# latk/hbetune.rs

Measured on NVIDIA B200. Metric: gp_fit_lml_evals_per_s, higher is better.
Workload: dtype f64

## Files before the change

### hbetune_rs_b200/csrc/gemm_i8.cuh

```cuda
#pragma once
#include <cuda.h>
#include <cuda_runtime.h>
#include <stdint.h>

#include "kernels.cuh"
#include "tcgen05.cuh"

namespace hbegp {
namespace oz {

using namespace tc;

constexpr int S = 14;
__host__ __device__ constexpr int modulus(int m) {
    return m == 0 ? 256 : m == 1 ? 255 : m == 2 ? 253 : m == 3 ? 251 : m == 4 ? 247 : m == 5 ? 241 : m == 6 ? 239
         : m == 7 ? 233 : m == 8 ? 229 : m == 9 ? 227 : m == 10 ? 223 : m == 11 ? 217 : m == 12 ? 211 : 199;
}
constexpr uint64_t P_LO = 0x3bdc01086e91ad00ull, P_HI = 0x0000478ff11c7ad1ull;
constexpr uint64_t HALF_LO = 0x9dee00843748d680ull, HALF_HI = 0x000023c7f88e3d68ull;
constexpr double INV_P58 = 1.9858025962649873e-16;
__host__ __device__ constexpr uint32_t crt_limb(int m, int l) {
    constexpr uint32_t t[S][4] = {
        {0x37fb0e01u, 0x3da6cc26u, 0xcdd91dc0u, 0x00000a57u},
        {0x2d9b6200u, 0x515b4421u, 0x61efbe69u, 0x00003c0eu},
        {0x6436c700u, 0xa8c49274u, 0x2ee81407u, 0x000033c3u},
        {0x0aaff900u, 0xaff19c1cu, 0xd136bce2u, 0x00000446u},
        {0xf7471500u, 0xd3598a93u, 0xb743daa4u, 0x000032b3u},
        {0xb4ac3100u, 0x80994803u, 0x38e00b2au, 0x00003a7fu},
        {0xb50dfd00u, 0xf9cd4608u, 0xfc396104u, 0x00001c71u},
        {0x0fc58900u, 0xf5ef92cau, 0x53de92a8u, 0x00002dc3u},
        {0x2b43a200u, 0x4f7c9d74u, 0xf258b82cu, 0x0000419fu},
        {0x93d41700u, 0x4d8fc60du, 0xcd5da098u, 0x0000303bu},
        {0x1a5f8a00u, 0x9a05c78eu, 0x5ab66f28u, 0x0000421bu},
        {0x5e122800u, 0x90ded2a3u, 0x9f5e87f5u, 0x00002cd9u},
        {0xd7195400u, 0xa67b8783u, 0xca9cace9u, 0x00003a55u},
        {0x8f385a00u, 0x80e799d2u, 0x8574cdfdu, 0x00003310u},
    };
    return t[m][l];
}

constexpr int TB = 128;
constexpr int TILE_BYTES = TB * TB;
constexpr int STAGES = 3;
constexpr int THREADS = 192;
constexpr int TMEM_COLS = 128;
constexpr size_t SMEM_BYTES = (size_t)STAGES * 2 * TILE_BYTES + 1024  + 256 ;
constexpr int E_CLAMP = 400;
constexpr int E_BAD = -32768;
constexpr int MAX_BITS = 50;

inline int scale_bits(int np) {
    const unsigned __int128 half = ((unsigned __int128)HALF_HI << 64) | HALF_LO;
    int b = MAX_BITS;
    while (b > 0 && ((unsigned __int128)np << (2 * b)) >= half) --b;
    return b;
}

__host__ __device__ inline long ntri_of(int tiles) { return (long)tiles * (tiles + 1) / 2; }
inline long ntri(int np) { return ntri_of((np + TB - 1) / TB); }
inline size_t slot_bytes(int np) {
    const size_t ex = ((size_t)(np + TB - 1) / TB * TB * sizeof(int) + TILE_BYTES - 1) / TILE_BYTES * TILE_BYTES;
    return 2 * (size_t)S * ntri(np) * TILE_BYTES + ex;
}

template <int M>
__device__ __forceinline__ uint32_t residue_byte(uint32_t lo24, uint32_t h0, uint32_t h1) {
    constexpr uint32_t p = (uint32_t)modulus(M);
    constexpr uint32_t c24 = (uint32_t)((1ull << 24) % p), c36 = (uint32_t)((1ull << 36) % p);
    constexpr uint32_t off = (uint32_t)(p - (uint32_t)((1ull << 51) % p));
    const uint32_t t = lo24 + h0 * c24 + h1 * c36 + off;
    uint32_t r = t % p;
    if (r > (p - 1) / 2) r -= p;
    return r & 0xffu;
}

template <int M>
__device__ __forceinline__ void store_residues(unsigned char* dst, const uint32_t (&lo)[16], const uint32_t (&h0)[16],
                                               const uint32_t (&h1)[16]) {
    uint32_t w[4];
#pragma unroll
    for (int q = 0; q < 4; q++)
        w[q] = residue_byte<M>(lo[4 * q], h0[4 * q], h1[4 * q]) | residue_byte<M>(lo[4 * q + 1], h0[4 * q + 1], h1[4 * q + 1]) << 8 |
               residue_byte<M>(lo[4 * q + 2], h0[4 * q + 2], h1[4 * q + 2]) << 16 |
               residue_byte<M>(lo[4 * q + 3], h0[4 * q + 3], h1[4 * q + 3]) << 24;
    *reinterpret_cast<uint4*>(dst) = make_uint4(w[0], w[1], w[2], w[3]);
}

template <int M>
__device__ __forceinline__ void store_all(unsigned char* dst, size_t plane_bytes, const uint32_t (&lo)[16], const uint32_t (&h0)[16],
                                          const uint32_t (&h1)[16]) {
    store_residues<M>(dst + (size_t)M * plane_bytes, lo, h0, h1);
    if constexpr (M + 1 < S) store_all<M + 1>(dst, plane_bytes, lo, h0, h1);
}

__global__ void __launch_bounds__(512) k_oz_colexp(const double* __restrict__ W, long mstride, int np, int bits,
                                                   unsigned char* __restrict__ ws, size_t slot) {
    __shared__ double smax[512];
    const int c = blockIdx.x, b = blockIdx.z, tid = threadIdx.x, col = tid & (TB - 1), ph = tid >> 7;
    const int nt = (np + TB - 1) / TB;
    const double* Wb = W + (long)b * mstride;
    int* ex = reinterpret_cast<int*>(ws + (size_t)b * slot + 2 * (size_t)S * ntri_of(nt) * TILE_BYTES);
    const int j = c * TB + col;
    double m = 0.0;
    if (j < np) {
        for (int k = c * TB + ph; k < min(np, (c + 1) * TB); k += 4)
            if (k >= j) { const double a = fabs(Wb[(long)k * np + j]); m = (a > m || a != a) ? a : m; }
#pragma unroll 8
        for (int k = (c + 1) * TB + ph; k < np; k += 4) { const double a = fabs(Wb[(long)k * np + j]); m = (a > m || a != a) ? a : m; }
    }
    smax[tid] = m;
    __syncthreads();
    if (tid < TB) {
        for (int q = 1; q < 4; q++) { const double a = smax[tid + q * TB]; m = (a > m || a != a) ? a : m; }
        int e = 0;
        if (!(m <= 0x1p+440)) {
            e = E_BAD;
        } else if (m > 0.0) {
            int E;
            frexp(m, &E);
            e = min(max(bits - E, -E_CLAMP), E_CLAMP);
        }
        ex[j] = e;
    }
}

__global__ void __launch_bounds__(256, 2) k_oz_split(const double* __restrict__ W, long mstride, int np,
                                                     unsigned char* __restrict__ ws, size_t slot) {
    int kb, c;
    lower_tile(blockIdx.x, kb, c);
    const int b = blockIdx.z, tid = threadIdx.x, col = tid & (TB - 1), j = c * TB + col;
    const long nr = ntri_of((np + TB - 1) / TB);
    const double* Wb = W + (long)b * mstride;
    unsigned char* wsb = ws + (size_t)b * slot;
    const int e = reinterpret_cast<const int*>(wsb + 2 * (size_t)S * nr * TILE_BYTES)[j];
    const double sc = e == E_BAD ? 0.0 : __longlong_as_double((long long)(1023 + e) << 52);
    const size_t plane_bytes = (size_t)nr * TILE_BYTES;
    unsigned char* tile = wsb + (size_t)blockIdx.x * TILE_BYTES;
    constexpr double MAGIC = 0x1.8p+52;
    for (int it = tid; it < TB * (TB / 16); it += 256) {
        const int ch = it >> 7, k0 = kb * TB + ch * 16;
        uint32_t lo[16], h0[16], h1[16];
#pragma unroll
        for (int q = 0; q < 16; q++) {
            const int k = k0 + q;
            const double w = (j < np && k < np && k >= j) ? Wb[(long)k * np + j] : 0.0;
            const uint64_t u = (uint64_t)__double_as_longlong(fma(w, sc, MAGIC)) & ((1ull << 52) - 1);
            lo[q] = (uint32_t)u & 0xffffffu;
            h0[q] = (uint32_t)(u >> 24) & 0xfffu;
            h1[q] = (uint32_t)(u >> 36);
        }
        store_all<0>(tile + (size_t)col * TB + ch * 16, plane_bytes, lo, h0, h1);
    }
}

struct SyrkParams {
    CUtensorMap map;
    unsigned char* ws;
    size_t slot;
    int nt;
    int slot_tiles;
};

constexpr uint32_t IDESC = (2u << 4) | (1u << 7) | (1u << 10) | ((uint32_t)(TB >> 3) << 17) | ((uint32_t)(TB >> 4) << 24);

__device__ __forceinline__ void mma_i8(uint32_t tmem_d, uint64_t adesc, uint64_t bdesc, uint32_t accumulate) {
    asm volatile(
        "{\n\t"
        ".reg .pred p;\n\t"
        "setp.ne.b32 p, %4, 0;\n\t"
        "tcgen05.mma.cta_group::1.kind::i8 [%0], %1, %2, %3, p;\n\t"
        "}\n" ::"r"(tmem_d),
        "l"(adesc), "l"(bdesc), "r"(IDESC), "r"(accumulate)
        : "memory");
}

__global__ void __launch_bounds__(THREADS, 2) k_oz_syrk_i8(const __grid_constant__ SyrkParams p) {
    extern __shared__ unsigned char smem_raw[];
    unsigned char* smem = reinterpret_cast<unsigned char*>((reinterpret_cast<uintptr_t>(smem_raw) + 1023) & ~(uintptr_t)1023);
    uint64_t* bars = reinterpret_cast<uint64_t*>(smem + (size_t)STAGES * 2 * TILE_BYTES);
    uint64_t* full = bars;
    uint64_t* empty = bars + STAGES;
    uint64_t* accf = bars + 2 * STAGES;
    uint32_t* tmem_slot = reinterpret_cast<uint32_t*>(accf + 1);

    const int tid = threadIdx.x, warp = tid >> 5, lane = tid & 31;
    int mt, nt;
    lower_tile(blockIdx.x, mt, nt);
    const int mod = blockIdx.y, bz = blockIdx.z;
    const long nr = (long)p.nt * (p.nt + 1) / 2;
    const int nk = p.nt - mt;
    const bool diag = mt == nt;

    if (warp == 0 && lane == 0) {
        for (int s = 0; s < STAGES; s++) {
            mbar_init(&full[s], 1);
            mbar_init(&empty[s], 1);
        }
        mbar_init(accf, 1);
        asm volatile("fence.mbarrier_init.release.cluster;" ::: "memory");
        asm volatile("prefetch.tensormap [%0];" ::"l"(reinterpret_cast<uint64_t>(&p.map)) : "memory");
    }
    if (warp == 1) {
        asm volatile("tcgen05.alloc.cta_group::1.sync.aligned.shared::cta.b32 [%0], %1;" ::"r"(smem_u32(tmem_slot)), "r"(TMEM_COLS)
                     : "memory");
        asm volatile("tcgen05.relinquish_alloc_permit.cta_group::1.sync.aligned;" ::: "memory");
    }
    asm volatile("tcgen05.fence::before_thread_sync;" ::: "memory");
    __syncthreads();
    asm volatile("tcgen05.fence::after_thread_sync;" ::: "memory");
    const uint32_t tmem_base = *tmem_slot;

    if (warp == 0) {
        if (lane == 0) {
            const int z0 = bz * p.slot_tiles + mod * (int)nr;
            for (int kt = 0; kt < nk; kt++) {
                const int s = kt % STAGES, kb = mt + kt;
                mbar_wait(&empty[s], ((kt / STAGES) & 1) ^ 1);
                unsigned char* st = smem + (size_t)s * 2 * TILE_BYTES;
                const int z = z0 + kb * (kb + 1) / 2;
                mbar_expect_tx(&full[s], diag ? TILE_BYTES : 2 * TILE_BYTES);
                tma_load_3d(&p.map, &full[s], st, 0, 0, z + mt);
                if (!diag) tma_load_3d(&p.map, &full[s], st + TILE_BYTES, 0, 0, z + nt);
            }
        }
    } else if (warp == 1) {
        if (lane == 0) {
            for (int kt = 0; kt < nk; kt++) {
                const int s = kt % STAGES;
                mbar_wait(&full[s], (kt / STAGES) & 1);
                asm volatile("tcgen05.fence::after_thread_sync;" ::: "memory");
                const uint32_t a = smem_u32(smem + (size_t)s * 2 * TILE_BYTES), bb = diag ? a : a + TILE_BYTES;
#pragma unroll
                for (int ks = 0; ks < TB / 32; ks++)
                    mma_i8(tmem_base, make_desc(a + 32 * ks, 16, 1024, 2), make_desc(bb + 32 * ks, 16, 1024, 2), (kt | ks) ? 1u : 0u);
                mma_commit(&empty[s]);
            }
            mma_commit(accf);
        }
    } else {
        const int lane_base = 32 * (warp & 3), row = lane_base + lane;
        const uint32_t lane_addr = tmem_base + ((uint32_t)lane_base << 16);
        const int pm = modulus(mod);
        const float inv = 1.0f / (float)pm;
        mbar_wait(accf, 0);
        asm volatile("tcgen05.fence::after_thread_sync;" ::: "memory");
        unsigned char* dst = p.ws + (size_t)bz * p.slot + ((size_t)(S + mod) * nr + blockIdx.x) * TILE_BYTES + (size_t)row * TB;
#pragma unroll
        for (int c0 = 0; c0 < TB; c0 += 32) {
            uint32_t v[32];
            tmem_ld32(lane_addr + c0, v);
            asm volatile("tcgen05.wait::ld.sync.aligned;" ::: "memory");
            uint32_t w[8];
#pragma unroll
            for (int q = 0; q < 8; q++) {
                uint32_t packed = 0;
#pragma unroll
                for (int e = 0; e < 4; e++) {
                    const int x = (int)v[4 * q + e];
                    int r = x - (int)floorf((float)x * inv) * pm;
                    r += r < 0 ? pm : 0;
                    r -= r >= pm ? pm : 0;
                    packed |= (uint32_t)r << (8 * e);
                }
                w[q] = packed;
            }
            reinterpret_cast<uint4*>(dst + c0)[0] = make_uint4(w[0], w[1], w[2], w[3]);
            reinterpret_cast<uint4*>(dst + c0)[1] = make_uint4(w[4], w[5], w[6], w[7]);
        }
        asm volatile("tcgen05.fence::before_thread_sync;" ::: "memory");
    }
    __syncthreads();
    if (warp == 1) {
        asm volatile("tcgen05.dealloc.cta_group::1.sync.aligned.b32 %0, %1;" ::"r"(tmem_base), "r"(TMEM_COLS) : "memory");
    }
}

__device__ __forceinline__ double crt_value(const uint32_t (&r)[S], int e) {
    uint64_t acc0 = 0, acc1 = 0, acc2 = 0, acc3 = 0;
#pragma unroll
    for (int m = 0; m < S; m++) {
        acc0 += (uint64_t)r[m] * crt_limb(m, 0);
        acc1 += (uint64_t)r[m] * crt_limb(m, 1);
        acc2 += (uint64_t)r[m] * crt_limb(m, 2);
        acc3 += (uint64_t)r[m] * crt_limb(m, 3);
    }
    typedef unsigned __int128 u128;
    typedef __int128 i128;
    const u128 sum = (u128)acc0 + ((u128)acc1 << 32) + ((u128)acc2 << 64) + ((u128)acc3 << 96);
    const u128 P = ((u128)P_HI << 64) | P_LO, half = ((u128)HALF_HI << 64) | HALF_LO;
    const uint32_t q = (uint32_t)((double)(uint64_t)(sum >> 58) * INV_P58);
    i128 v = (i128)(sum - (u128)q * P);
    if (v < 0) v += (i128)P;
    if (v >= (i128)P) v -= (i128)P;
    if (v > (i128)half) v -= (i128)P;
    const bool neg = v < 0;
    const u128 a = neg ? (u128)(-v) : (u128)v;
    const uint64_t hi = (uint64_t)(a >> 64), lo = (uint64_t)a;
    double d;
    int sh = 0;
    if (hi == 0) {
        d = __ull2double_rn(lo);
    } else {
        sh = 64 - __clzll((long long)hi);
        const uint64_t mant = (uint64_t)(a >> sh) | ((lo & ((1ull << sh) - 1)) != 0 ? 1ull : 0ull);
        d = __ull2double_rn(mant);
    }
    d *= __longlong_as_double((long long)(1023 + sh - e) << 52);
    return neg ? -d : d;
}

__global__ void __launch_bounds__(256) k_oz_merge(double* __restrict__ C, long mstride, int np, const unsigned char* __restrict__ ws,
                                                  size_t slot) {
    int mt, nt;
    lower_tile(blockIdx.x, mt, nt);
    const int b = blockIdx.z, tnum = (np + TB - 1) / TB;
    const long nr = (long)tnum * (tnum + 1) / 2;
    const unsigned char* wsb = ws + (size_t)b * slot;
    const unsigned char* res = wsb + ((size_t)S * nr + blockIdx.x) * TILE_BYTES;
    const int* ex = reinterpret_cast<const int*>(wsb + 2 * (size_t)S * nr * TILE_BYTES);
    double* Cb = C + (long)b * mstride;
    for (int it = threadIdx.x; it < TB * TB / 4; it += 256) {
        const int row = it >> 5, c4 = (it & 31) * 4;
        const int gi = mt * TB + row, gj = nt * TB + c4;
        if (gi >= np || gj >= np) continue;
        if (mt == nt && (row >> 6) < (c4 >> 6)) continue;
        uint32_t w[S];
#pragma unroll
        for (int m = 0; m < S; m++) w[m] = *reinterpret_cast<const uint32_t*>(res + (size_t)m * nr * TILE_BYTES + row * TB + c4);
        const int ei = ex[gi];
        const int4 ej = *reinterpret_cast<const int4*>(ex + gj);
        const int ejs[4] = {ej.x, ej.y, ej.z, ej.w};
        double out[4];
#pragma unroll
        for (int q = 0; q < 4; q++) {
            uint32_t r[S];
#pragma unroll
            for (int m = 0; m < S; m++) r[m] = (w[m] >> (8 * q)) & 0xffu;
            out[q] = (ei == E_BAD || ejs[q] == E_BAD) ? __longlong_as_double(0x7ff8000000000000ll) : crt_value(r, ei + ejs[q]);
        }
        double2* dst = reinterpret_cast<double2*>(Cb + (long)gi * np + gj);
        dst[0] = make_double2(out[0], out[1]);
        dst[1] = make_double2(out[2], out[3]);
    }
}

inline cudaError_t configure() {
    return cudaFuncSetAttribute(k_oz_syrk_i8, cudaFuncAttributeMaxDynamicSharedMemorySize, (int)SMEM_BYTES);
}

inline cudaError_t launch_kinv(const double* W, double* C, long mstride, int np, int cnt, unsigned char* ws, cudaStream_t st) {
    if (cnt <= 0) return cudaSuccess;
    const int tn = (np + TB - 1) / TB;
    const size_t slot = slot_bytes(np);
    k_oz_colexp<<<dim3(tn, 1, cnt), 512, 0, st>>>(W, mstride, np, scale_bits(np), ws, slot);
    k_oz_split<<<dim3((unsigned)ntri(np), 1, cnt), 256, 0, st>>>(W, mstride, np, ws, slot);
    cudaError_t e = cudaGetLastError();
    if (e != cudaSuccess) return e;
    SyrkParams p;
    p.ws = ws;
    p.slot = slot;
    p.nt = tn;
    p.slot_tiles = (int)(slot / TILE_BYTES);
    EncodeTiledFn enc = encode_fn();
    if (!enc) return cudaErrorNotSupported;
    cuuint64_t dims[3] = {(cuuint64_t)TB, (cuuint64_t)TB, (cuuint64_t)p.slot_tiles * cnt};
    cuuint64_t strides[2] = {(cuuint64_t)TB, (cuuint64_t)TILE_BYTES};
    cuuint32_t box[3] = {(cuuint32_t)TB, (cuuint32_t)TB, 1};
    cuuint32_t estr[3] = {1, 1, 1};
    if (enc(&p.map, CU_TENSOR_MAP_DATA_TYPE_UINT8, 3, ws, dims, strides, box, estr, CU_TENSOR_MAP_INTERLEAVE_NONE,
            CU_TENSOR_MAP_SWIZZLE_128B, CU_TENSOR_MAP_L2_PROMOTION_L2_256B, CU_TENSOR_MAP_FLOAT_OOB_FILL_NONE) != CUDA_SUCCESS)
        return cudaErrorNotSupported;
    k_oz_syrk_i8<<<dim3((unsigned)ntri(np), S, cnt), THREADS, SMEM_BYTES, st>>>(p);
    if ((e = cudaGetLastError()) != cudaSuccess) return e;
    k_oz_merge<<<dim3((unsigned)ntri(np), 1, cnt), 256, 0, st>>>(C, mstride, np, ws, slot);
    return cudaGetLastError();
}

}
}
```

### hbetune_rs_b200/csrc/hbegp.cu

```cuda
#include <cuda_runtime.h>

#include <algorithm>
#include <chrono>
#include <cmath>
#include <cstdio>
#include <cstdlib>
#include <cstring>
#include <functional>
#include <limits>
#include <condition_variable>
#include <map>
#include <mutex>
#include <string>
#include <thread>
#include <tuple>
#include <vector>

#include "../../include/hbegp.h"
#include "gemm.cuh"
#include "gemm_tf32.cuh"
#include "gemm_i8.cuh"
#include "kernels.cuh"
#include "node_mma.cuh"
#include "lbfgs.h"
// ... 336 lines not shown
        CUDA_TRY(cudaMemcpyAsync(dX.p, x, (size_t)n * d * sizeof(T), kind, stream));
        CUDA_TRY(cudaMemcpyAsync(dY.p, y, (size_t)n * sizeof(T), kind, stream));
        if (!on_device) CUDA_TRY(cudaStreamSynchronize(stream));
        return HBEGP_OK;
    }

    size_t per_slot_bytes() const {
        size_t s = 2 * (size_t)np * np * sizeof(T);
        s += (size_t)d * np * sizeof(T) + (size_t)p() * sizeof(T) + 2 * (size_t)np * sizeof(T);
        s += (size_t)(np / TILE) * sizeof(T) + (size_t)nchunks() * np * sizeof(T);
        s += (size_t)ntiles_lower() * p() * sizeof(double) + (size_t)(p() + 1) * sizeof(double) + sizeof(int);
        if (kinv_emulated()) s += oz::slot_bytes(np);
        return s;
    }

    int ensure_capacity(int want) {
        if (n <= 0) return fail(HBEGP_ERR_INVALID, "no training data: call hbegp_set_data first");
        if (want <= cap) return HBEGP_OK;
        size_t limit = ws_limit;
        size_t fr = 0, tot = 0;
        CUDA_TRY(cudaMemGetInfo(&fr, &tot));
        const size_t held = A.bytes + W.bytes + gpart.bytes + tpart.bytes + xsT.bytes + oz.bytes;
        if (limit == 0) limit = (size_t)((double)(fr + held + model_pool.held) * 0.7);
        size_t per = per_slot_bytes();
        int fit = (int)std::min<size_t>(limit / per, 4096);
        if (fit < 1) return fail(HBEGP_ERR_NOMEM, "workspace limit too small for one n x n evaluation");
        int newcap = std::min(want, fit);
        if (newcap <= cap) return HBEGP_OK;
        if ((size_t)newcap * per > fr + held) model_pool.clear();
        drop_graphs();
        int rc;
        size_t c = (size_t)newcap;
        if ((rc = A.ensure(c * np * np * sizeof(T)))) return rc;
        if ((rc = W.ensure(c * np * np * sizeof(T)))) return rc;
        if ((rc = xsT.ensure(c * d * np * sizeof(T)))) return rc;
        if ((rc = prm.ensure(c * p() * sizeof(T)))) return rc;
        if ((rc = u.ensure(c * np * sizeof(T)))) return rc;
        if ((rc = alpha.ensure(c * np * sizeof(T)))) return rc;
        if ((rc = ldp.ensure(c * (np / TILE) * sizeof(T)))) return rc;
        if ((rc = tpart.ensure(c * nchunks() * np * sizeof(T)))) return rc;
        if ((rc = gpart.ensure(c * ntiles_lower() * p() * sizeof(double)))) return rc;
        if ((rc = d_lml.ensure(c * sizeof(double)))) return rc;
        if ((rc = d_grad.ensure(c * p() * sizeof(double)))) return rc;
        if ((rc = d_status.ensure(((size_t)c + 1) * sizeof(int)))) return rc;
        if (kinv_emulated() && (rc = oz.ensure(c * oz::slot_bytes(np)))) return rc;
        if (h_prm_bytes < c * p() * sizeof(T)) {
            if (h_prm) cudaFreeHost(h_prm);
            h_prm_bytes = c * p() * sizeof(T);
            CUDA_TRY(cudaMallocHost((void**)&h_prm, h_prm_bytes));
        }
        if (h_out_bytes < c * (p() + 1) * sizeof(double)) {
            if (h_out) cudaFreeHost(h_out);
            h_out_bytes = c * (p() + 1) * sizeof(double);
            CUDA_TRY(cudaMallocHost((void**)&h_out, h_out_bytes));
        }
        if (h_status_bytes < c * sizeof(int)) {
            if (h_status) cudaFreeHost(h_status);
            h_status_bytes = c * sizeof(int);
            CUDA_TRY(cudaMallocHost((void**)&h_status, h_status_bytes));
        }
        cap = newcap;
        return HBEGP_OK;
    }

    void fill_params(const double* theta, const double* lo, const double* hi, T* out) const {
        out[0] = (T)std::exp(theta[0]);
        for (int k = 1; k < p(); k++) {
            double v = std::exp(theta[k]);
            if (lo && v < lo[k]) v = lo[k];
            else if (hi && hi[k] < v) v = hi[k];
            out[k] = (T)v;
        }
    }

    struct Side {
        cudaStream_t st = nullptr;
        cudaEvent_t a = nullptr, b = nullptr;
    };

    int chol_inv(cudaStream_t st, int s0, int cnt, int r0, int s, Side sd = Side()) {
        T* Ab = (T*)A.p + (size_t)s0 * mstride();
        T* Wb = (T*)W.p + (size_t)s0 * mstride();
        if (s == TILE) {
            CUDA_TRY(launch_prio(k_leaf<T>, dim3(1, 1, cnt), dim3(256), leaf_smem_bytes<T>(), st, Ab, Wb, mstride(), np, r0,
                                 (T*)ldp.p + (size_t)s0 * (np / TILE), np / TILE, (int*)d_status.p + s0));
            launches++;
            return HBEGP_OK;
        }
        if (s == 2 * TILE) {
            CUDA_TRY(launch_prio(k_node128_v2<false, T>, dim3(1, 1, cnt), dim3(256), node128_v2_smem_bytes(), st, Ab, Wb, mstride(), np, r0,
                                 (T*)ldp.p + (size_t)s0 * (np / TILE), np / TILE, (int*)d_status.p + s0, (long long*)nullptr));
            launches++;
            return HBEGP_OK;
        }
        int q = s / TILE, q1 = (q + 1) / 2;
        if (q >= 4 && (q1 & 1)) q1 += 1;
        if (q1 >= q) q1 = q - 1;
        const int s1 = q1 * TILE, s2 = s - s1;
        int rc;
        if ((rc = chol_inv(st, s0, cnt, r0, s1, sd))) return rc;
        return merge_node(st, s0, cnt, r0, s1, s2, sd);
    }

    int merge_node(cudaStream_t st, int s0, int cnt, int r0, int s1, int s2, Side sd) {
        T* Ab = (T*)A.p + (size_t)s0 * mstride();
        T* Wb = (T*)W.p + (size_t)s0 * mstride();
        int rc;
        T* A21 = Ab + (long)(r0 + s1) * np + r0;
        T* W21 = Wb + (long)(r0 + s1) * np + r0;
        T* W11 = Wb + (long)r0 * np + r0;
        T* A22 = Ab + (long)(r0 + s1) * np + r0 + s1;
        T* W22 = Wb + (long)(r0 + s1) * np + r0 + s1;
        GemmArgs<T> g{};
        g.lda = g.ldb = g.ldc = np;
        g.sA = g.sB = g.sC = mstride();
        g.rowsumsq = nullptr;
        g.small_ctas = np <= SMALL_TILE_NP ? SMALL_TILE_CTAS : 0;
        g.A = A21; g.B = W11; g.C = W21; g.M = s2; g.N = s1; g.K = s1; g.kmode = K_LE_N; g.lower_only = 0;
        g.alpha = T(1); g.beta = T(0);
        CUDA_TRY((launch_gemm_auto<T, true, true>(g, cnt, st))); launches++;
        cudaStream_t st3 = st;
        if (sd.st) {
            CUDA_TRY(cudaEventRecord(sd.a, st));
            CUDA_TRY(cudaStreamWaitEvent(sd.st, sd.a, 0));
            st3 = sd.st;
        }
        g.A = W21; g.B = W11; g.C = A21; g.M = s2; g.N = s1; g.K = s1; g.kmode = K_GE_N; g.lower_only = 0;
        g.alpha = T(1); g.beta = T(0);
        CUDA_TRY((launch_gemm_auto<T, true, false>(g, cnt, st3))); launches++;
        if (sd.st) CUDA_TRY(cudaEventRecord(sd.b, sd.st));
        g.A = W21; g.B = W21; g.C = A22; g.M = s2; g.N = s2; g.K = s1; g.kmode = K_FULL; g.lower_only = 1;
        g.alpha = T(-1); g.beta = T(1);
        CUDA_TRY((launch_gemm_auto<T, true, true>(g, cnt, st))); launches++;
        if ((rc = chol_inv(st, s0, cnt, r0 + s1, s2, sd))) return rc;
        if (sd.st) CUDA_TRY(cudaStreamWaitEvent(st, sd.b, 0));
        g.A = W22; g.B = A21; g.C = W21; g.M = s2; g.N = s1; g.K = s2; g.kmode = K_LE_M; g.lower_only = 0;
        g.alpha = T(-1); g.beta = T(0);
        CUDA_TRY((launch_gemm_auto<T, true, false>(g, cnt, st))); launches++;
        return HBEGP_OK;
    }

    static constexpr long SMALL_TILE_CTAS = 296;
    static constexpr int SMALL_TILE_NP = 1024;

    static constexpr int OZ_MIN_NP = 2048;
    bool kinv_emulated() const { return std::is_same<T, double>::value && np >= OZ_MIN_NP; }

    int lauum(cudaStream_t st, int s0, int cnt) {
        T* Ab = (T*)A.p + (size_t)s0 * mstride();
        T* Wb = (T*)W.p + (size_t)s0 * mstride();
        if constexpr (std::is_same<T, double>::value) {
            if (kinv_emulated()) {
                CUDA_TRY(oz::launch_kinv(Wb, Ab, mstride(), np, cnt, (unsigned char*)oz.p + (size_t)s0 * oz::slot_bytes(np), st));
                launches += 4;
                return HBEGP_OK;
            }
        }
        GemmArgs<T> g{};
        g.lda = g.ldb = g.ldc = np;
        g.sA = g.sB = g.sC = mstride();
        g.A = Wb; g.B = Wb; g.C = Ab; g.M = np; g.N = np; g.K = np; g.kmode = K_GE_M; g.lower_only = 1;
        g.alpha = T(1); g.beta = T(0);
        g.rowsumsq = nullptr;
        g.small_ctas = np <= SMALL_TILE_NP ? SMALL_TILE_CTAS : 0;
        CUDA_TRY((launch_gemm_auto<T, false, false>(g, cnt, st))); launches++;
        return HBEGP_OK;
    }

    int phase = 3;

    template <int NU2>
    int pipeline_nu(cudaStream_t st, int s0, int cnt, bool want_grad, bool want_kinv, Side sd) {
        T* Ab = (T*)A.p + (size_t)s0 * mstride();
        T* Wb = (T*)W.p + (size_t)s0 * mstride();
        T* xs = (T*)xsT.p + (size_t)s0 * d * np;
        T* pr = (T*)prm.p + (size_t)s0 * p();
        T* ub = (T*)u.p + (size_t)s0 * np;
        T* al = (T*)alpha.p + (size_t)s0 * np;
        T* tp = (T*)tpart.p + (size_t)s0 * nchunks() * np;
        double* gp = (double*)gpart.p + (size_t)s0 * ntiles_lower() * p();
        const size_t xsm = 2 * (size_t)feat_chunk(d) * TILE * sizeof(T);
        if (phase == 5) return lauum(st, s0, cnt);
        k_scale_x<T><<<dim3((np + 255) / 256, d, cnt), 256, 0, st>>>((const T*)dX.p, (int)n, d, np, pr, p(), xs);
        launches++;
        k_assemble<T, NU2><<<dim3(ntiles_lower(), 1, cnt), 256, xsm, st>>>(xs, (int)n, d, np, pr, p(), Ab, mstride(), 0);
        launches++;
        CUDA_TRY(cudaGetLastError());
        if (phase < 1) return HBEGP_OK;
        int rc;
        if ((rc = chol_inv(st, s0, cnt, 0, np, sd))) return rc;
        if (phase < 2) return HBEGP_OK;
        const bool split = sd.st && (want_grad || want_kinv);
        cudaStream_t sa = st;
        if (split) {
            CUDA_TRY(cudaEventRecord(sd.a, st));
            CUDA_TRY(cudaStreamWaitEvent(sd.st, sd.a, 0));
            sa = sd.st;
        }
        k_trmv_lower<T><<<dim3(np / 8, 1, cnt), 256, 0, sa>>>(Wb, mstride(), np, (const T*)dY.p, 0, ub, np);
        launches++;
        k_trmv_lower_t_part<T><<<dim3(np / TILE, nchunks(), cnt), 256, 0, sa>>>(Wb, mstride(), np, ub, np, tp, nchunks());
        launches++;
        CUDA_TRY(launch_prio(k_sum_chunks<T>, dim3((np + 255) / 256, 1, cnt), dim3(256), 0, sa, tp, nchunks(), np, al, (long)np));
        launches++;
        if (split) CUDA_TRY(cudaEventRecord(sd.b, sd.st));
        if (want_grad || want_kinv) {
            if ((rc = lauum(st, s0, cnt))) return rc;
        }
        if (split) CUDA_TRY(cudaStreamWaitEvent(st, sd.b, 0));
        if (phase < 3) return HBEGP_OK;
        if (want_grad) {
            const size_t gsm = xsm + 2 * TILE * sizeof(T) + 8 * (size_t)(feat_chunk(d) + 2) * sizeof(double);
            k_grad_contract<T, NU2><<<dim3(ntiles_lower(), 1, cnt), 256, gsm, st>>>(
                Ab, mstride(), (int)n, d, np, xs, al, np, pr, p(), gp, (long)ntiles_lower() * p());
            launches++;
        }
        CUDA_TRY(launch_prio(k_finish<T>, dim3(cnt), dim3(256), 0, st, (const T*)dY.p, al, np, (int)n, np, (T*)ldp.p + (size_t)s0 * (np / TILE),
                             np / TILE, gp, (long)ntiles_lower() * p(), ntiles_lower(), p(), (int*)d_status.p + s0, (double*)d_lml.p + s0,
                             (double*)d_grad.p + (size_t)s0 * p(), want_grad ? 1 : 0));
        launches++;
        return HBEGP_OK;
    }

    int pipeline(int nu2, cudaStream_t st, int s0, int cnt, bool want_grad, bool want_kinv, Side sd = Side()) {
        constexpr int SIDE_MAX_CNT = 4;
        if (!((np <= 2048 || cnt <= SIDE_MAX_CNT) && np > TILE)) sd = Side();
        if (nu2 == 5) return pipeline_nu<5>(st, s0, cnt, want_grad, want_kinv, sd);
        if (nu2 == 3) return pipeline_nu<3>(st, s0, cnt, want_grad, want_kinv, sd);
        return pipeline_nu<1>(st, s0, cnt, want_grad, want_kinv, sd);
    }

    int n_groups(int cnt) const {
        int g = (int)sub.size();
        const int gm = np >= 1024 ? 1 : 2;
        if (np <= 2048) g = std::min(g, std::max(1, cnt / gm));
        else g = std::min(g, 4);
        return std::max(1, std::min(g, cnt));
    }

    int issue_chunk(int nu2, int cnt, bool want_grad, bool want_kinv) {
        CUDA_TRY(cudaMemcpyAsync(prm.p, h_prm, (size_t)cnt * p() * sizeof(T), cudaMemcpyHostToDevice, stream));
        CUDA_TRY(cudaMemsetAsync(d_status.p, 0, (size_t)cnt * sizeof(int), stream));
        const int groups = n_groups(cnt);
        if (groups <= 1) {
            Side sd;
            sd.st = main_side; sd.a = main_a; sd.b = main_b;
            int rc = pipeline(nu2, stream, 0, cnt, want_grad, want_kinv, sd);
            if (rc) return rc;
        } else {
            CUDA_TRY(cudaEventRecord(fork_ev, stream));
            int base = cnt / groups, extra = cnt % groups, s0 = 0;
            for (int g = 0; g < groups; g++) {
                int c = base + (g < extra ? 1 : 0);
                CUDA_TRY(cudaStreamWaitEvent(sub[g], fork_ev, 0));
                Side sd;
                sd.st = side[g]; sd.a = side_a[g]; sd.b = side_b[g];
                int rc = pipeline(nu2, sub[g], s0, c, want_grad, want_kinv, sd);
                if (rc) return rc;
                CUDA_TRY(cudaEventRecord(sub_done[g], sub[g]));
                CUDA_TRY(cudaStreamWaitEvent(stream, sub_done[g], 0));
                s0 += c;
            }
        }
        CUDA_TRY(cudaMemcpyAsync(h_out, d_lml.p, (size_t)cnt * sizeof(double), cudaMemcpyDeviceToHost, stream));
        if (want_grad)
            CUDA_TRY(cudaMemcpyAsync(h_out + cap, d_grad.p, (size_t)cnt * p() * sizeof(double), cudaMemcpyDeviceToHost, stream));
        CUDA_TRY(cudaMemcpyAsync(h_status, d_status.p, (size_t)cnt * sizeof(int), cudaMemcpyDeviceToHost, stream));
        return HBEGP_OK;
    }

    int run_chunk(int nu2, int cnt, bool want_grad, bool want_kinv) {
        const bool legacy = (stream == nullptr || stream == cudaStreamLegacy);
        if (legacy || np > 2048) {
            int rc = issue_chunk(nu2, cnt, want_grad, want_kinv);
            if (rc) return rc;
            CUDA_TRY(cudaStreamSynchronize(stream));
            return HBEGP_OK;
        }
        auto key = std::make_tuple(nu2, cnt, (int)want_grad, (int)want_kinv, phase);
        auto it = graphs.find(key);
        if (it == graphs.end() || it->second.epoch != graph_epoch) {
            const long long before = launches;
            const double t_cap = now_ms();
            CUDA_TRY(cudaStreamBeginCapture(stream, cudaStreamCaptureModeRelaxed));
            int rc = issue_chunk(nu2, cnt, want_grad, want_kinv);
            cudaGraph_t graph = nullptr;
            cudaError_t ce = cudaStreamEndCapture(stream, &graph);
            const long long kernels = launches - before;
            launches = before;
            if (rc) {
                if (graph) cudaGraphDestroy(graph);
                return rc;
            }
            if (ce != cudaSuccess) return fail(HBEGP_ERR_CUDA, std::string("cudaStreamEndCapture: ") + cudaGetErrorString(ce));
            bool updated = false;
            if (it != graphs.end()) {
                cudaGraphExecUpdateResultInfo info;
                if (cudaGraphExecUpdate(it->second.exec, graph, &info) == cudaSuccess) {
                    updated = true;
                    it->second.epoch = graph_epoch;
                    it->second.kernels = kernels;
                } else {
                    cudaGetLastError();
                    cudaGraphExecDestroy(it->second.exec);
                    graphs.erase(it);
                    it = graphs.end();
                }
// ... 1875 lines not shown
```

### probes/kinv_emul_bench.py

```python
import argparse
import json
import math
import os
import subprocess
import sys
import tempfile
import time

import numpy as np

ROOT = os.path.dirname(os.path.dirname(os.path.abspath(__file__)))
SIZES = (512, 768, 1024, 1536, 2048, 3072, 4096)
D = 16


def _data(n, seed=1):
    rng = np.random.default_rng(seed)
    x = rng.random((n, D))
    y = np.sin(2 * np.pi * x).sum(axis=1)
    y = (y - y.min()) / (y - y.min()).mean() + 0.05
    return x, y


def _thetas(B, noise):
    rng = np.random.default_rng(B)
    th = np.empty((B, D + 2))
    th[:, 0] = math.log(noise)
    th[:, 1] = rng.uniform(-0.5, 0.5, B)
    th[:, 2:] = np.log(rng.uniform(0.8, 2.0, (B, D)))
    return th


def worker(args):
    sys.path.insert(0, ROOT)
    import hbetune_rs_b200 as h

    out = {"lib": os.environ.get("HBEGP_LIB", "")}
    if args.timing:
        rows = []
        for n in SIZES:
            x, y = _data(n)
            with h.Context(0, h.F64) as ctx:
                ctx.set_data(x, y)
                for B in (1, 65):
                    th = _thetas(B, 1e-2)
                    step = ctx.bench_phase(th, 3, 3)
                    kinv = ctx.bench_phase(th, 5, 5)
                    rows.append({"n": n, "B": B, "step_ms": step, "kinv_ms": kinv})
        out["timing"] = rows
    if args.check:
        os.makedirs(args.check, exist_ok=True)
        tag = os.path.basename(os.path.dirname(out["lib"])) or "default"
        res = {}
        for n, noise in ((1100, 1e-2), (2049, 1e-4), (4096, 1e-2)):
            x, y = _data(n, seed=n)
            th = _thetas(3, noise)
            with h.Context(0, h.F64) as ctx:
                ctx.set_data(x, y)
                lml, grad, status = ctx.lml_grad_batch(th)
                m = ctx.model(th[0], want_alpha=True, want_kinv=True)
                res[f"n{n}_lml"], res[f"n{n}_grad"], res[f"n{n}_status"] = lml, grad, status
                res[f"n{n}_alpha"], res[f"n{n}_kinv"] = m.alpha, m.k_inv
        np.savez(os.path.join(args.check, f"{tag}.npz"), **res)
        out["check"] = os.path.join(args.check, f"{tag}.npz")
    print(json.dumps(out), flush=True)


def main():
    ap = argparse.ArgumentParser()
    ap.add_argument("--lib", action="append", default=[], help="name=path of a libhbegp.so")
    ap.add_argument("--rounds", type=int, default=3)
    ap.add_argument("--out", default="")
    ap.add_argument("--check-dir", default="", help="where the workers leave their outputs (default: a temporary directory)")
    ap.add_argument("--worker", action="store_true")
    ap.add_argument("--timing", action="store_true")
    ap.add_argument("--check", default="")
    args = ap.parse_args()
    if args.worker:
        return worker(args)
    libs = [tuple(s.split("=", 1)) for s in args.lib]
    check_dir = args.check_dir or tempfile.mkdtemp(prefix="kinv_emul_")
    runs = {name: [] for name, _ in libs}
    checks = {}
    for r in range(args.rounds):
        for name, path in libs:
            cmd = [sys.executable, __file__, "--worker", "--timing"]
            if r == 0:
                cmd += ["--check", os.path.join(check_dir, name)]
            t0 = time.perf_counter()
            p = subprocess.run(cmd, env=dict(os.environ, HBEGP_LIB=os.path.abspath(path)), capture_output=True, text=True)
            if p.returncode != 0:
                sys.exit(f"{name} round {r} failed:\n{p.stdout}\n{p.stderr}")
            rec = json.loads(p.stdout.strip().splitlines()[-1])
            if "check" in rec:
                checks[name] = rec["check"]
            runs[name].append(rec["timing"])
            print(f"{name} round {r}: {time.perf_counter() - t0:.1f} s", flush=True)
    summary = {}
    for name in runs:
        for i, row in enumerate(runs[name][0]):
            key = f"n={row['n']} B={row['B']}"
            ks = [rr[i]["kinv_ms"] for rr in runs[name]]
            ss = [rr[i]["step_ms"] for rr in runs[name]]
            summary.setdefault(key, {})[name] = {"kinv_ms": ks, "step_ms": ss}
    for key, v in summary.items():
        print(key, "  ".join(f"{nm}: kinv {min(x['kinv_ms']):.3f}-{max(x['kinv_ms']):.3f} ms step {min(x['step_ms']):.2f}-"
                             f"{max(x['step_ms']):.2f} ms" for nm, x in v.items()), flush=True)
    agree = {}
    if len(checks) == 2:
        (na, pa), (nb, pb) = checks.items()
        a, b = np.load(pa), np.load(pb)
        for k in a.files:
            if k.endswith(("_lml", "_alpha", "_status")):
                agree[k] = "identical" if np.array_equal(a[k], b[k]) else f"differs by {float(np.abs(a[k] - b[k]).max()):.3e}"
            else:
                agree[k] = float(np.abs(a[k] - b[k]).max() / np.abs(a[k]).max())
        for k, v in agree.items():
            print(f"{na} vs {nb} {k}: {v}", flush=True)
    if args.out:
        with open(args.out, "w") as f:
            json.dump({"timing": summary, "agreement": agree}, f, indent=1)


if __name__ == "__main__":
    main()
```

Before: 508.4.

## Pair SYRK output tiles, parallelize column-exponent scan, cheapen residue math

The int8 Ozaki SYRK kernel now computes two adjacent output tiles per block (128x256 accumulator in TMEM), loading one A tile and two B tiles per stage and using two stages instead of three. This reuses the A operand and halves the block count. The column-max pass is rebuilt as a per-tile kernel that atomicMaxes IEEE-exponent keys, plus a key-clear kernel, and split and merge decode the exponents from those keys. The residue modulo uses a multiply-high reciprocal with byte_perm packing, and the split loop covers 8 elements per item. This adds an extra kernel launch and atomics, and the larger accumulator uses more TMEM per block, which may reduce occupancy.

Result: faster. 527.7, median of 6 (+3.8%).

```diff
diff --git a/hbetune_rs_b200/csrc/gemm_i8.cuh b/hbetune_rs_b200/csrc/gemm_i8.cuh
--- a/hbetune_rs_b200/csrc/gemm_i8.cuh
+++ b/hbetune_rs_b200/csrc/gemm_i8.cuh
@@ -41,10 +41,11 @@
 
 constexpr int TB = 128;
 constexpr int TILE_BYTES = TB * TB;
-constexpr int STAGES = 3;
+constexpr int STAGES = 2;
+constexpr int STAGE_BYTES = 3 * TILE_BYTES;
 constexpr int THREADS = 192;
-constexpr int TMEM_COLS = 128;
-constexpr size_t SMEM_BYTES = (size_t)STAGES * 2 * TILE_BYTES + 1024  + 256 ;
+constexpr int TMEM_COLS = 256;
+constexpr size_t SMEM_BYTES = (size_t)STAGES * STAGE_BYTES + 1024  + 256 ;
 constexpr int E_CLAMP = 400;
 constexpr int E_BAD = -32768;
 constexpr int MAX_BITS = 50;
@@ -66,82 +67,84 @@
 template <int M>
 __device__ __forceinline__ uint32_t residue_byte(uint32_t lo24, uint32_t h0, uint32_t h1) {
     constexpr uint32_t p = (uint32_t)modulus(M);
-    constexpr uint32_t c24 = (uint32_t)((1ull << 24) % p), c36 = (uint32_t)((1ull << 36) % p);
+    if constexpr (p == 256) return lo24;
+    constexpr uint32_t c24 = (uint32_t)((1ull << 24) % p), c36 = (uint32_t)((1ull << 36) % p), h = (p - 1) / 2;
     constexpr uint32_t off = (uint32_t)(p - (uint32_t)((1ull << 51) % p));
-    const uint32_t t = lo24 + h0 * c24 + h1 * c36 + off;
-    uint32_t r = t % p;
-    if (r > (p - 1) / 2) r -= p;
-    return r & 0xffu;
+    constexpr uint32_t magic = (uint32_t)(((1ull << 39) + p - 1) / p);
+    const uint32_t t = lo24 + h0 * c24 + h1 * c36 + (off + h);
+    const uint32_t q = __umulhi(t, magic) >> 7;
+    return t - h - q * p;
 }
 
 template <int M>
-__device__ __forceinline__ void store_residues(unsigned char* dst, const uint32_t (&lo)[16], const uint32_t (&h0)[16],
-                                               const uint32_t (&h1)[16]) {
-    uint32_t w[4];
-#pragma unroll
-    for (int q = 0; q < 4; q++)
-        w[q] = residue_byte<M>(lo[4 * q], h0[4 * q], h1[4 * q]) | residue_byte<M>(lo[4 * q + 1], h0[4 * q + 1], h1[4 * q + 1]) << 8 |
-               residue_byte<M>(lo[4 * q + 2], h0[4 * q + 2], h1[4 * q + 2]) << 16 |
-               residue_byte<M>(lo[4 * q + 3], h0[4 * q + 3], h1[4 * q + 3]) << 24;
-    *reinterpret_cast<uint4*>(dst) = make_uint4(w[0], w[1], w[2], w[3]);
+__device__ __forceinline__ void store_residues(unsigned char* dst, const uint32_t (&lo)[8], const uint32_t (&h0)[8], const uint32_t (&h1)[8]) {
+    uint32_t w[2];
+#pragma unroll
+    for (int q = 0; q < 2; q++)
+        w[q] = __byte_perm(__byte_perm(residue_byte<M>(lo[4 * q], h0[4 * q], h1[4 * q]), residue_byte<M>(lo[4 * q + 1], h0[4 * q + 1], h1[4 * q + 1]), 0x0040),
+                           __byte_perm(residue_byte<M>(lo[4 * q + 2], h0[4 * q + 2], h1[4 * q + 2]), residue_byte<M>(lo[4 * q + 3], h0[4 * q + 3], h1[4 * q + 3]), 0x0040),
+                           0x5410);
+    *reinterpret_cast<uint2*>(dst) = make_uint2(w[0], w[1]);
 }
 
 template <int M>
-__device__ __forceinline__ void store_all(unsigned char* dst, size_t plane_bytes, const uint32_t (&lo)[16], const uint32_t (&h0)[16],
-                                          const uint32_t (&h1)[16]) {
+__device__ __forceinline__ void store_all(unsigned char* dst, size_t plane_bytes, const uint32_t (&lo)[8], const uint32_t (&h0)[8],
+                                          const uint32_t (&h1)[8]) {
     store_residues<M>(dst + (size_t)M * plane_bytes, lo, h0, h1);
     if constexpr (M + 1 < S) store_all<M + 1>(dst, plane_bytes, lo, h0, h1);
 }
 
-__global__ void __launch_bounds__(512) k_oz_colexp(const double* __restrict__ W, long mstride, int np, int bits,
-                                                   unsigned char* __restrict__ ws, size_t slot) {
-    __shared__ double smax[512];
-    const int c = blockIdx.x, b = blockIdx.z, tid = threadIdx.x, col = tid & (TB - 1), ph = tid >> 7;
-    const int nt = (np + TB - 1) / TB;
-    const double* Wb = W + (long)b * mstride;
-    int* ex = reinterpret_cast<int*>(ws + (size_t)b * slot + 2 * (size_t)S * ntri_of(nt) * TILE_BYTES);
-    const int j = c * TB + col;
-    double m = 0.0;
-    if (j < np) {
-        for (int k = c * TB + ph; k < min(np, (c + 1) * TB); k += 4)
-            if (k >= j) { const double a = fabs(Wb[(long)k * np + j]); m = (a > m || a != a) ? a : m; }
-#pragma unroll 8
-        for (int k = (c + 1) * TB + ph; k < np; k += 4) { const double a = fabs(Wb[(long)k * np + j]); m = (a > m || a != a) ? a : m; }
-    }
-    smax[tid] = m;
-    __syncthreads();
-    if (tid < TB) {
-        for (int q = 1; q < 4; q++) { const double a = smax[tid + q * TB]; m = (a > m || a != a) ? a : m; }
-        int e = 0;
-        if (!(m <= 0x1p+440)) {
-            e = E_BAD;
-        } else if (m > 0.0) {
-            int E;
-            frexp(m, &E);
-            e = min(max(bits - E, -E_CLAMP), E_CLAMP);
-        }
-        ex[j] = e;
-    }
-}
-
-__global__ void __launch_bounds__(256, 2) k_oz_split(const double* __restrict__ W, long mstride, int np,
-                                                     unsigned char* __restrict__ ws, size_t slot) {
+__global__ void __launch_bounds__(256) k_oz_colexp(const double* __restrict__ W, long mstride, int np, unsigned char* __restrict__ ws,
+                                                   size_t slot) {
     int kb, c;
     lower_tile(blockIdx.x, kb, c);
-    const int b = blockIdx.z, tid = threadIdx.x, col = tid & (TB - 1), j = c * TB + col;
+    const int b = blockIdx.z, tid = threadIdx.x, j = c * TB + (tid & (TB - 1));
+    if (j >= np) return;
+    const double* Wb = W + (long)b * mstride;
+    unsigned* key = reinterpret_cast<unsigned*>(ws + (size_t)b * slot + 2 * (size_t)S * ntri_of((np + TB - 1) / TB) * TILE_BYTES);
+    const int r0 = kb * TB + (tid >> 7) * (TB / 2), k1 = min(r0 + TB / 2, np);
+    unsigned m = 0;
+#pragma unroll 8
+    for (int k = max(r0, j); k < k1; k++) {
+        const unsigned long long u = (unsigned long long)__double_as_longlong(Wb[(long)k * np + j]) & 0x7fffffffffffffffull;
+        m = max(m, (unsigned)(u >> 32) | ((unsigned)u != 0u ? 1u : 0u));
+    }
+    if (m) atomicMax(key + j, m);
+}
+
+__global__ void __launch_bounds__(TB) k_oz_keyclear(int np, unsigned char* __restrict__ ws, size_t slot) {
+    unsigned* key = reinterpret_cast<unsigned*>(ws + (size_t)blockIdx.z * slot + 2 * (size_t)S * ntri_of((np + TB - 1) / TB) * TILE_BYTES);
+    key[blockIdx.x * TB + threadIdx.x] = 0u;
+}
+
+__device__ __forceinline__ int col_exp(unsigned key, int bits) {
+    if (key > 0x5b700000u) return E_BAD;
+    if (key == 0u) return 0;
+    if (key < 0x00100000u) return E_CLAMP;
+    return min(max(bits - ((int)(key >> 20) - 1022), -E_CLAMP), E_CLAMP);
+}
+
+__global__ void __launch_bounds__(256) k_oz_split(const double* __restrict__ W, long mstride, int np, int bits,
+                                                  unsigned char* __restrict__ ws, size_t slot) {
+    int kb, c;
+    lower_tile(blockIdx.x, kb, c);
+    const int b = blockIdx.z, tid = threadIdx.x;
     const long nr = ntri_of((np + TB - 1) / TB);
     const double* Wb = W + (long)b * mstride;
     unsigned char* wsb = ws + (size_t)b * slot;
-    const int e = reinterpret_cast<const int*>(wsb + 2 * (size_t)S * nr * TILE_BYTES)[j];
-    const double sc = e == E_BAD ? 0.0 : __longlong_as_double((long long)(1023 + e) << 52);
+    const unsigned* key = reinterpret_cast<const unsigned*>(wsb + 2 * (size_t)S * nr * TILE_BYTES);
     const size_t plane_bytes = (size_t)nr * TILE_BYTES;
     unsigned char* tile = wsb + (size_t)blockIdx.x * TILE_BYTES;
     constexpr double MAGIC = 0x1.8p+52;
-    for (int it = tid; it < TB * (TB / 16); it += 256) {
-        const int ch = it >> 7, k0 = kb * TB + ch * 16;
-        uint32_t lo[16], h0[16], h1[16];
-#pragma unroll
-        for (int q = 0; q < 16; q++) {
+#pragma unroll 1
+    for (int it = tid; it < TB * (TB / 8); it += 256) {
+        const int col = (it >> 6) * 4 + ((it >> 3) & 3), kc = ((it >> 5) & 1) * 8 + (it & 7);
+        const int j = c * TB + col, k0 = kb * TB + kc * 8;
+        const int e = col_exp(key[j], bits);
+        const double sc = e == E_BAD ? 0.0 : __longlong_as_double((long long)(1023 + e) << 52);
+        uint32_t lo[8], h0[8], h1[8];
+#pragma unroll
+        for (int q = 0; q < 8; q++) {
             const int k = k0 + q;
             const double w = (j < np && k < np && k >= j) ? Wb[(long)k * np + j] : 0.0;
             const uint64_t u = (uint64_t)__double_as_longlong(fma(w, sc, MAGIC)) & ((1ull << 52) - 1);
@@ -149,7 +152,7 @@
             h0[q] = (uint32_t)(u >> 24) & 0xfffu;
             h1[q] = (uint32_t)(u >> 36);
         }
-        store_all<0>(tile + (size_t)col * TB + ch * 16, plane_bytes, lo, h0, h1);
+        store_all<0>(tile + (size_t)col * TB + kc * 8, plane_bytes, lo, h0, h1);
     }
 }
 
@@ -161,35 +164,47 @@
     int slot_tiles;
 };
 
-constexpr uint32_t IDESC = (2u << 4) | (1u << 7) | (1u << 10) | ((uint32_t)(TB >> 3) << 17) | ((uint32_t)(TB >> 4) << 24);
-
-__device__ __forceinline__ void mma_i8(uint32_t tmem_d, uint64_t adesc, uint64_t bdesc, uint32_t accumulate) {
+__host__ __device__ constexpr uint32_t idesc(int n) {
+    return (2u << 4) | (1u << 7) | (1u << 10) | ((uint32_t)(n >> 3) << 17) | ((uint32_t)(TB >> 4) << 24);
+}
+
+__device__ __forceinline__ void mma_i8(uint32_t tmem_d, uint64_t adesc, uint64_t bdesc, uint32_t id, uint32_t accumulate) {
     asm volatile(
         "{\n\t"
         ".reg .pred p;\n\t"
         "setp.ne.b32 p, %4, 0;\n\t"
         "tcgen05.mma.cta_group::1.kind::i8 [%0], %1, %2, %3, p;\n\t"
         "}\n" ::"r"(tmem_d),
-        "l"(adesc), "l"(bdesc), "r"(IDESC), "r"(accumulate)
+        "l"(adesc), "l"(bdesc), "r"(id), "r"(accumulate)
         : "memory");
+}
+
+__host__ __device__ inline long nblocks_of(int tiles) { return (long)((tiles + 1) / 2) * (tiles / 2 + 1); }
+__device__ __forceinline__ void pair_block(int t, int& mt, int& J) {
+    int a = (int)((sqrtf(4.0f * (float)t + 1.0f) - 1.0f) * 0.5f);
+    while ((a + 1) * (a + 2) <= t) ++a;
+    while (a * (a + 1) > t) --a;
+    if (t < (a + 1) * (a + 1)) { mt = 2 * a; J = t - a * (a + 1); }
+    else { mt = 2 * a + 1; J = t - (a + 1) * (a + 1); }
 }
 
 __global__ void __launch_bounds__(THREADS, 2) k_oz_syrk_i8(const __grid_constant__ SyrkParams p) {
     extern __shared__ unsigned char smem_raw[];
     unsigned char* smem = reinterpret_cast<unsigned char*>((reinterpret_cast<uintptr_t>(smem_raw) + 1023) & ~(uintptr_t)1023);
-    uint64_t* bars = reinterpret_cast<uint64_t*>(smem + (size_t)STAGES * 2 * TILE_BYTES);
+    uint64_t* bars = reinterpret_cast<uint64_t*>(smem + (size_t)STAGES * STAGE_BYTES);
     uint64_t* full = bars;
     uint64_t* empty = bars + STAGES;
     uint64_t* accf = bars + 2 * STAGES;
     uint32_t* tmem_slot = reinterpret_cast<uint32_t*>(accf + 1);
 
     const int tid = threadIdx.x, warp = tid >> 5, lane = tid & 31;
-    int mt, nt;
-    lower_tile(blockIdx.x, mt, nt);
+    int mt, J;
+    pair_block(blockIdx.x, mt, J);
     const int mod = blockIdx.y, bz = blockIdx.z;
     const long nr = (long)p.nt * (p.nt + 1) / 2;
     const int nk = p.nt - mt;
-    const bool diag = mt == nt;
+    const bool diag = 2 * J == mt;
+    const int ncols = diag ? TB : 2 * TB;
 
     if (warp == 0 && lane == 0) {
         for (int s = 0; s < STAGES; s++) {
@@ -216,23 +231,27 @@
             for (int kt = 0; kt < nk; kt++) {
                 const int s = kt % STAGES, kb = mt + kt;
                 mbar_wait(&empty[s], ((kt / STAGES) & 1) ^ 1);
-                unsigned char* st = smem + (size_t)s * 2 * TILE_BYTES;
+                unsigned char* st = smem + (size_t)s * STAGE_BYTES;
                 const int z = z0 + kb * (kb + 1) / 2;
-                mbar_expect_tx(&full[s], diag ? TILE_BYTES : 2 * TILE_BYTES);
+                mbar_expect_tx(&full[s], diag ? TILE_BYTES : 3 * TILE_BYTES);
                 tma_load_3d(&p.map, &full[s], st, 0, 0, z + mt);
-                if (!diag) tma_load_3d(&p.map, &full[s], st + TILE_BYTES, 0, 0, z + nt);
+                if (!diag) {
+                    tma_load_3d(&p.map, &full[s], st + TILE_BYTES, 0, 0, z + 2 * J);
+                    tma_load_3d(&p.map, &full[s], st + 2 * TILE_BYTES, 0, 0, z + 2 * J + 1);
+                }
             }
         }
     } else if (warp == 1) {
         if (lane == 0) {
+            const uint32_t id = idesc(ncols);
             for (int kt = 0; kt < nk; kt++) {
                 const int s = kt % STAGES;
                 mbar_wait(&full[s], (kt / STAGES) & 1);
                 asm volatile("tcgen05.fence::after_thread_sync;" ::: "memory");
-                const uint32_t a = smem_u32(smem + (size_t)s * 2 * TILE_BYTES), bb = diag ? a : a + TILE_BYTES;
+                const uint32_t a = smem_u32(smem + (size_t)s * STAGE_BYTES), bb = diag ? a : a + TILE_BYTES;
 #pragma unroll
                 for (int ks = 0; ks < TB / 32; ks++)
-                    mma_i8(tmem_base, make_desc(a + 32 * ks, 16, 1024, 2), make_desc(bb + 32 * ks, 16, 1024, 2), (kt | ks) ? 1u : 0u);
+                    mma_i8(tmem_base, make_desc(a + 32 * ks, 16, 1024, 2), make_desc(bb + 32 * ks, 16, 1024, 2), id, (kt | ks) ? 1u : 0u);
                 mma_commit(&empty[s]);
             }
             mma_commit(accf);
@@ -244,9 +263,10 @@
         const float inv = 1.0f / (float)pm;
         mbar_wait(accf, 0);
         asm volatile("tcgen05.fence::after_thread_sync;" ::: "memory");
-        unsigned char* dst = p.ws + (size_t)bz * p.slot + ((size_t)(S + mod) * nr + blockIdx.x) * TILE_BYTES + (size_t)row * TB;
-#pragma unroll
-        for (int c0 = 0; c0 < TB; c0 += 32) {
+        unsigned char* dst = p.ws + (size_t)bz * p.slot + ((size_t)(S + mod) * nr + (size_t)mt * (mt + 1) / 2 + 2 * J) * TILE_BYTES +
+                             (size_t)row * TB;
+#pragma unroll 1
+        for (int c0 = 0; c0 < ncols; c0 += 32) {
             uint32_t v[32];
             tmem_ld32(lane_addr + c0, v);
             asm volatile("tcgen05.wait::ld.sync.aligned;" ::: "memory");
@@ -264,8 +284,9 @@
                 }
                 w[q] = packed;
             }
-            reinterpret_cast<uint4*>(dst + c0)[0] = make_uint4(w[0], w[1], w[2], w[3]);
-            reinterpret_cast<uint4*>(dst + c0)[1] = make_uint4(w[4], w[5], w[6], w[7]);
+            unsigned char* d = dst + (c0 >= TB ? TILE_BYTES : 0) + (c0 & (TB - 1));
+            reinterpret_cast<uint4*>(d)[0] = make_uint4(w[0], w[1], w[2], w[3]);
+            reinterpret_cast<uint4*>(d)[1] = make_uint4(w[4], w[5], w[6], w[7]);
         }
         asm volatile("tcgen05.fence::before_thread_sync;" ::: "memory");
     }
@@ -309,16 +330,19 @@
     return neg ? -d : d;
 }
 
-__global__ void __launch_bounds__(256) k_oz_merge(double* __restrict__ C, long mstride, int np, const unsigned char* __restrict__ ws,
-                                                  size_t slot) {
+__global__ void __launch_bounds__(256) k_oz_merge(double* __restrict__ C, long mstride, int np, int bits,
+                                                  const unsigned char* __restrict__ ws, size_t slot) {
     int mt, nt;
     lower_tile(blockIdx.x, mt, nt);
     const int b = blockIdx.z, tnum = (np + TB - 1) / TB;
     const long nr = (long)tnum * (tnum + 1) / 2;
     const unsigned char* wsb = ws + (size_t)b * slot;
     const unsigned char* res = wsb + ((size_t)S * nr + blockIdx.x) * TILE_BYTES;
-    const int* ex = reinterpret_cast<const int*>(wsb + 2 * (size_t)S * nr * TILE_BYTES);
+    const unsigned* key = reinterpret_cast<const unsigned*>(wsb + 2 * (size_t)S * nr * TILE_BYTES);
     double* Cb = C + (long)b * mstride;
+    __shared__ __align__(16) int ex[2 * TB];
+    ex[threadIdx.x] = col_exp(key[(threadIdx.x < TB ? mt : nt) * TB + (threadIdx.x & (TB - 1))], bits);
+    __syncthreads();
     for (int it = threadIdx.x; it < TB * TB / 4; it += 256) {
         const int row = it >> 5, c4 = (it & 31) * 4;
         const int gi = mt * TB + row, gj = nt * TB + c4;
@@ -327,8 +351,8 @@
         uint32_t w[S];
 #pragma unroll
         for (int m = 0; m < S; m++) w[m] = *reinterpret_cast<const uint32_t*>(res + (size_t)m * nr * TILE_BYTES + row * TB + c4);
-        const int ei = ex[gi];
-        const int4 ej = *reinterpret_cast<const int4*>(ex + gj);
+        const int ei = ex[row];
+        const int4 ej = *reinterpret_cast<const int4*>(ex + TB + c4);
         const int ejs[4] = {ej.x, ej.y, ej.z, ej.w};
         double out[4];
 #pragma unroll
@@ -350,10 +374,11 @@
 
 inline cudaError_t launch_kinv(const double* W, double* C, long mstride, int np, int cnt, unsigned char* ws, cudaStream_t st) {
     if (cnt <= 0) return cudaSuccess;
-    const int tn = (np + TB - 1) / TB;
+    const int tn = (np + TB - 1) / TB, bits = scale_bits(np);
     const size_t slot = slot_bytes(np);
-    k_oz_colexp<<<dim3(tn, 1, cnt), 512, 0, st>>>(W, mstride, np, scale_bits(np), ws, slot);
-    k_oz_split<<<dim3((unsigned)ntri(np), 1, cnt), 256, 0, st>>>(W, mstride, np, ws, slot);
+    k_oz_keyclear<<<dim3(tn, 1, cnt), TB, 0, st>>>(np, ws, slot);
+    k_oz_colexp<<<dim3((unsigned)ntri(np), 1, cnt), 256, 0, st>>>(W, mstride, np, ws, slot);
+    k_oz_split<<<dim3((unsigned)ntri(np), 1, cnt), 256, 0, st>>>(W, mstride, np, bits, ws, slot);
     cudaError_t e = cudaGetLastError();
     if (e != cudaSuccess) return e;
     SyrkParams p;
@@ -370,9 +395,9 @@
     if (enc(&p.map, CU_TENSOR_MAP_DATA_TYPE_UINT8, 3, ws, dims, strides, box, estr, CU_TENSOR_MAP_INTERLEAVE_NONE,
             CU_TENSOR_MAP_SWIZZLE_128B, CU_TENSOR_MAP_L2_PROMOTION_L2_256B, CU_TENSOR_MAP_FLOAT_OOB_FILL_NONE) != CUDA_SUCCESS)
         return cudaErrorNotSupported;
-    k_oz_syrk_i8<<<dim3((unsigned)ntri(np), S, cnt), THREADS, SMEM_BYTES, st>>>(p);
+    k_oz_syrk_i8<<<dim3((unsigned)nblocks_of(tn), S, cnt), THREADS, SMEM_BYTES, st>>>(p);
     if ((e = cudaGetLastError()) != cudaSuccess) return e;
-    k_oz_merge<<<dim3((unsigned)ntri(np), 1, cnt), 256, 0, st>>>(C, mstride, np, ws, slot);
+    k_oz_merge<<<dim3((unsigned)ntri(np), 1, cnt), 256, 0, st>>>(C, mstride, np, bits, ws, slot);
     return cudaGetLastError();
 }
 
diff --git a/hbetune_rs_b200/csrc/hbegp.cu b/hbetune_rs_b200/csrc/hbegp.cu
--- a/hbetune_rs_b200/csrc/hbegp.cu
+++ b/hbetune_rs_b200/csrc/hbegp.cu
@@ -512,7 +512,7 @@
         if constexpr (std::is_same<T, double>::value) {
             if (kinv_emulated()) {
                 CUDA_TRY(oz::launch_kinv(Wb, Ab, mstride(), np, cnt, (unsigned char*)oz.p + (size_t)s0 * oz::slot_bytes(np), st));
-                launches += 4;
+                launches += 5;
                 return HBEGP_OK;
             }
         }
diff --git a/probes/kinv_emul_bench.py b/probes/kinv_emul_bench.py
--- a/probes/kinv_emul_bench.py
+++ b/probes/kinv_emul_bench.py
@@ -36,6 +36,25 @@
     import hbetune_rs_b200 as h
 
     out = {"lib": os.environ.get("HBEGP_LIB", "")}
+    if args.kernels:
+        import torch
+        from torch.profiler import ProfilerActivity, profile
+
+        n, B, reps = 4096, 65, 5
+        x, y = _data(n)
+        with h.Context(0, h.F64) as ctx:
+            ctx.set_data(x, y)
+            th = _thetas(B, 1e-2)
+            ctx.bench_phase(th, 3, 2)
+            ctx.bench_phase(th, 5, 2)
+            with profile(activities=[ProfilerActivity.CUDA]) as prof:
+                ctx.bench_phase(th, 5, reps)
+        ks = {}
+        for ev in prof.key_averages():
+            if "oz" in ev.key:
+                name = ev.key.split("(")[0].split("::")[-1]
+                ks[name] = ks.get(name, 0.0) + ev.device_time_total / 1e3 / reps
+        out["kernels_ms"] = ks
     if args.timing:
         rows = []
         for n in SIZES:
@@ -66,6 +85,32 @@
     print(json.dumps(out), flush=True)
 
 
+def floors_ms(n=4096, B=65, S=14):
+    t = n // 128
+    lower = t * (t + 1) // 2
+    macs = sum((t - mt) * (mt + 1) for mt in range(t)) * 128 ** 3 * S * B
+    w = lower * 128 * 128 * 8 * B
+    planes = S * lower * 128 * 128 * B
+    return {"k_oz_syrk_i8": 2 * macs / 4.5e15 * 1e3, "k_oz_split": (w + planes) / 7.7e12 * 1e3,
+            "k_oz_merge": (planes + w) / 7.7e12 * 1e3, "k_oz_colexp": w / 7.7e12 * 1e3}
+
+
+def kernels(libs, out_path):
+    res = {}
+    for name, path in libs:
+        p = subprocess.run([sys.executable, __file__, "--worker", "--kernels"], env=dict(os.environ, HBEGP_LIB=os.path.abspath(path)),
+                           capture_output=True, text=True)
+        if p.returncode != 0:
+            sys.exit(f"{name} failed:\n{p.stdout}\n{p.stderr}")
+        res[name] = json.loads(p.stdout.strip().splitlines()[-1])["kernels_ms"]
+    fl = floors_ms()
+    for k in sorted({k for r in res.values() for k in r}):
+        print(f"{k:14s}", "  ".join(f"{nm} {r.get(k, 0.0):7.3f} ms" for nm, r in res.items()), f"  floor {fl.get(k, 0.0):6.3f} ms", flush=True)
+    if out_path:
+        with open(out_path, "w") as f:
+            json.dump({"kernels_ms": res, "floor_ms": fl, "shape": "n = 4096, B = 65, per phase-5 launch sequence"}, f, indent=1)
+
+
 def main():
     ap = argparse.ArgumentParser()
     ap.add_argument("--lib", action="append", default=[], help="name=path of a libhbegp.so")
@@ -75,10 +120,13 @@
     ap.add_argument("--worker", action="store_true")
     ap.add_argument("--timing", action="store_true")
     ap.add_argument("--check", default="")
+    ap.add_argument("--kernels", action="store_true", help="per-kernel times of the K^-1 launches (torch.profiler)")
     args = ap.parse_args()
     if args.worker:
         return worker(args)
     libs = [tuple(s.split("=", 1)) for s in args.lib]
+    if args.kernels:
+        return kernels(libs, args.out)
     check_dir = args.check_dir or tempfile.mkdtemp(prefix="kinv_emul_")
     runs = {name: [] for name, _ in libs}
     checks = {}
```
